# sndels/yuki

Measured on AMD Instinct MI355X. Metric: Mray/s (primary+secondary), Path integrator @1080p, higher is better.
Workload: dtype f32; 1 GPU; cfg3: city 40x20 displaced icospheres, 1,024,012 triangles, SAH BVH (max_shapes_in_node 1), Path 8 bounces, Stratified 8x8, 1920x1080; triangles=1024012, spp=64, max_depth=8, tiles=8160, partition=single GPU, frames_in_flight=2

## Files before the change

yuki_amd/csrc/yk_kernels.h:

```cpp
#pragma once
#include <hip/hip_runtime.h>

#include "yk_device.h"

namespace yk {

unsigned trace_block_size();
unsigned trace_spill_depth();
unsigned trace_top_nodes();
unsigned trace_top_nodes_any();
unsigned packet_blocks_per_cu();
void launch_trace_closest_packet(hipStream_t s, unsigned grid, const DevScene& sc, const float4* rayO, const float4* rayD, const unsigned* count_ptr,
                                 unsigned* head, int* hit_tri, unsigned long long* ray_counter, const float4* lean_origin = nullptr, CancelRef cancel = CancelRef{nullptr, nullptr});
void launch_trace_any_packet(hipStream_t s, unsigned grid, const DevScene& sc, const float4* shO, const float4* shD, const unsigned* slot_of,
                             const unsigned* count_ptr, unsigned* head, unsigned char* vis, unsigned long long* shadow_counter, CancelRef cancel = CancelRef{nullptr, nullptr});
unsigned trace_blocks_per_cu();

void launch_pixel_table(hipStream_t s, const yk_tile* tiles, const uint32_t* tile_offset, uint32_t n_tiles, uint32_t n_pixels, uint32_t* pixel_xy,
                        const uint16_t* tile_sample = nullptr, uint32_t* pixel_sample = nullptr);
void launch_pixel_table_one(hipStream_t s, const yk_tile& tile, uint32_t n_pixels, uint32_t* pixel_xy, uint32_t tile_sample, uint32_t* pixel_sample);
void launch_raygen(hipStream_t s, const DevCamera& cam, const RenderParams& prm, const uint32_t* pixel_xy, const uint32_t* pixel_sample, uint64_t work0,
                   uint32_t n, PathBuffers out, float4* sample_buf, unsigned* count, float4* lean_origin = nullptr, const uint4* pixel_aux = nullptr);
void launch_pixel_sampler(hipStream_t s, const SamplerCfg& cfg, const uint32_t* pixel_xy, uint32_t n_pixels, uint4* pixel_aux);
void launch_raygen_user(hipStream_t s, const RenderParams& prm, const float* o, const float* d, const uint16_t* pixel, const uint32_t* sample_index,
                        uint32_t dimension, uint32_t n, PathBuffers out, float4* sample_buf, uint32_t* pixel_xy, unsigned* ctrl);
void launch_trace_closest(hipStream_t s, unsigned grid, const DevScene& sc, const float4* rayO, const float4* rayD, const float* t_max_opt,
                          const unsigned* count_ptr, unsigned* head, int* hit_tri, float4* hit_out, uint4* stats_out, uint2* spill,
                          unsigned spill_stride, unsigned* ctrl, unsigned long long* ray_counter, const unsigned* cancel_host = nullptr);
void launch_whitted(hipStream_t s, unsigned grid, const DevScene& sc, const RenderParams& prm, const uint32_t* pixel_xy, const uint32_t* sample_index_tab,
                    PathBuffers cur, uint32_t n, float4* sample_buf, uint2* spill, unsigned spill_stride, unsigned* ctrl, unsigned long long* counters);
unsigned whitted_max_depth();
void launch_path_debug(hipStream_t s, unsigned grid, const DevScene& sc, const RenderParams& prm, const uint32_t* pixel_xy, const uint32_t* sample_index_tab,
                       PathBuffers cur, uint32_t n, float4* sample_buf, uint32_t* out_counts, float4* out_rays, unsigned ray_cap, uint32_t* out_n_rays,
                       float min_len, uint2* spill, unsigned spill_stride, unsigned* ctrl);
void launch_trace_any(hipStream_t s, unsigned grid, const DevScene& sc, const float4* shO, const float4* shD, const unsigned* slot_of,
                      const unsigned* count_ptr, unsigned* head, unsigned char* vis, uint2* spill, unsigned spill_stride, unsigned* ctrl,
                      unsigned long long* shadow_counter, const unsigned* cancel_host = nullptr);
void launch_shade(hipStream_t s, unsigned grid, const DevScene& sc, const RenderParams& prm, const uint32_t* pixel_xy, const uint32_t* sample_index_tab,
                  PathBuffers cur, PathBuffers nxt, const int* hit_tri, float4* pend, float4* shO, float4* shD, float4* shC, unsigned char* vis,
                  unsigned* shq, float4* shO2, float4* shD2, unsigned* shq2, unsigned* bc, unsigned split_delta, unsigned reorder, unsigned block_slots, unsigned sid_base, const float4* lean_origin);
void launch_accumulate(hipStream_t s, unsigned grid, const RenderParams& prm, PathBuffers cur, const float4* pend, const float4* shC,
                       const unsigned char* vis, unsigned nl, float4* sample_buf, const unsigned* bc, unsigned first, unsigned sid_base);
void launch_resolve(hipStream_t s, const float4* sample_buf, uint32_t n_pixels, uint32_t spp, float* out_rgb);
void launch_resolve_passes(hipStream_t s, const float4* sample_buf, uint32_t n_pixels, uint32_t n_passes, float* out_rgb, size_t pass_stride);
void launch_film_scatter(hipStream_t s, const uint32_t* pixel_xy, uint32_t n_pixels, const float* tile_rgb, uint32_t res_x, float* film_rgb, int accumulate,
                         uint32_t n_passes = 1, size_t pass_stride = 0);
void launch_debug_shade(hipStream_t s, const DevScene& sc, uint32_t integrator, PathBuffers cur, const int* hit_tri, const uint4* stats, uint32_t n,
                        float4* sample_buf);
void launch_device_math(hipStream_t s, int fn, size_t n, const float* a, const float* b, float* out);
void launch_sampler_sequence(hipStream_t s, const SamplerCfg& cfg, uint32_t px, uint32_t py, uint32_t sample_index, const uint8_t* dims, size_t n_draws,
                             float* out);
void launch_light_test(hipStream_t s, const DevLight& L, int index, size_t n, const float* p, const float* ng, const float* u, float* out);
void launch_bsdf_test(hipStream_t s, const Material& m, size_t n, const float* ng, const float* ns, const float* dpdu, const float* wo,
                      const float* wi_or_u, int sample, float* out);
void launch_pack_rays(hipStream_t s, size_t n, const float* o, const float* d, float4* rayO, float4* rayD);
void launch_pack_shadow_rays(hipStream_t s, size_t n, const float* o, const float* d, const float* t_max, const int* area_light, float4* shO,
                             float4* shD);
void launch_unpack_rays(hipStream_t s, size_t n, const float4* rayO, const float4* rayD, float* o, float* d);

}
```

yuki_amd/csrc/yk_kernels.hip:

```cpp
#include <hip/hip_runtime.h>

#include "yk_device.h"
#include "yk_geom.h"
#include "yk_kernels.h"
#include "yk_rng.h"
#include "yk_shade.h"
#include "yk_wave.h"

namespace yk {

__global__ void k_pixel_table(const yk_tile* tiles, const uint32_t* tile_offset, uint32_t n_tiles, uint32_t n_pixels,
                              uint32_t* pixel_xy, const uint16_t* tile_sample, uint32_t* pixel_sample) {
    uint32_t i = blockIdx.x * blockDim.x + threadIdx.x;
    if (i >= n_pixels) return;
    uint32_t lo = 0, hi = n_tiles;
    while (hi - lo > 1) {
        uint32_t mid = (lo + hi) >> 1;
        if (tile_offset[mid] <= i)
            lo = mid;
        else
            hi = mid;
    }
    yk_tile t = tiles[lo];
    uint32_t w = (uint32_t)t.x1 - t.x0;
    uint32_t r = i - tile_offset[lo];
    uint32_t x = t.x0 + r % w, y = t.y0 + r / w;
    pixel_xy[i] = x | (y << 16);
    if (tile_sample) pixel_sample[i] = tile_sample[lo];
}

__global__ void k_pixel_table_one(yk_tile t, uint32_t n_pixels, uint32_t* pixel_xy, uint32_t tile_sample, uint32_t* pixel_sample) {
    uint32_t i = blockIdx.x * blockDim.x + threadIdx.x;
    if (i >= n_pixels) return;
    uint32_t w = (uint32_t)t.x1 - t.x0;
    pixel_xy[i] = (t.x0 + i % w) | ((t.y0 + i / w) << 16);
    if (pixel_sample) pixel_sample[i] = tile_sample;
}

__global__ void k_pixel_sampler(SamplerCfg cfg, const uint32_t* pixel_xy, uint32_t n_pixels, uint4* pixel_aux) {
    uint32_t i = blockIdx.x * blockDim.x + threadIdx.x;
    if (i >= n_pixels) return;
    const uint32_t xy = pixel_xy[i];
    const PixelSampler ps = pixel_sampler(cfg, xy & 0xffffu, xy >> 16);
    pixel_aux[i] = make_uint4((unsigned)ps.stream, (unsigned)(ps.stream >> 32), ps.hash0, 0u);
}

__device__ __forceinline__ void camera_ray(const DevCamera& cam, float fx, float fy, V3& o, V3& d) {
    V3 p_camera = xf_point(cam.r2c, V3{fx, fy, 0.0f});
    V3 dir = normalize(p_camera);
    o = xf_point(cam.c2w, V3{0.0f, 0.0f, 0.0f});
    d = xf_vector(cam.c2w, dir);
}

__global__ void k_raygen(DevCamera cam, RenderParams prm, const uint32_t* pixel_xy, const uint32_t* pixel_sample, uint64_t work0, uint32_t n,
                         PathBuffers out, float4* sample_buf, unsigned* count, float4* lean_origin, const uint4* pixel_aux) {
    uint32_t i = blockIdx.x * blockDim.x + threadIdx.x;
    if (cancel_raised(prm.cancel)) return;
    if (i == 0) *count = n;
    if (i >= n) return;
    const uint32_t w = (uint32_t)(work0 + i);
    uint32_t pix, ks;
    split_sample_id(w, prm.spe, pix, ks);
    const uint32_t s = (pixel_sample ? pixel_sample[pix] : prm.sample_base) + ks;
    uint32_t xy = pixel_xy[pix];
    uint32_t px = xy & 0xffffu, py = xy >> 16;
    SamplerState st;
    float ux, uy;
    if (pixel_aux) {
        const uint4 a = pixel_aux[pix];
        PixelSampler ps;
        ps.stream = (u64)a.x | ((u64)a.y << 32);
        ps.hash0 = a.z;
        st = sampler_start_camera(prm.sampler, ps, px, py, s, ux, uy);
    } else {
        st = sampler_start(prm.sampler, px, py, s, 0);
        sampler_get_2d(prm.sampler, st, ux, uy);
    }
    V3 o, d;
    camera_ray(cam, (float)px + ux, (float)py + uy, o, d);
    if (lean_origin) {
        if (i == 0) *lean_origin = make_float4(o.x, o.y, o.z, __uint_as_float(0u));
    } else {
        out.rayO[i] = make_float4(o.x, o.y, o.z, __uint_as_float(0u));
        out.thru[i] = make_float4(1.0f, 1.0f, 1.0f, __uint_as_float(st.dimension));
    }
    out.rayD[i] = make_float4(d.x, d.y, d.z, __uint_as_float((uint32_t)w));
    out.rngs[i] = make_uint4((unsigned)st.rng.state, (unsigned)(st.rng.state >> 32), (unsigned)st.rng.inc, (unsigned)(st.rng.inc >> 32));
    if (prm.integrator != YK_INTEGRATOR_PATH || prm.max_depth == 0) sample_buf[w] = make_float4(0.0f, 0.0f, 0.0f, 0.0f);
}

__global__ void k_raygen_user(RenderParams prm, const float* ray_o, const float* ray_d, const uint16_t* pixel, const uint32_t* sample_index,
                              uint32_t dimension, uint32_t n, PathBuffers out, float4* sample_buf, uint32_t* pixel_xy, unsigned* count) {
    uint32_t i = blockIdx.x * blockDim.x + threadIdx.x;
    if (i == 0) *count = n;
    if (i >= n) return;
    uint32_t px = pixel[2 * i], py = pixel[2 * i + 1];
    pixel_xy[i] = px | (py << 16);
    SamplerState st = sampler_start(prm.sampler, px, py, sample_index[i], dimension);
    if (prm.sampler.kind == 1) st.dimension = dimension;
    out.rayO[i] = make_float4(ray_o[3 * i], ray_o[3 * i + 1], ray_o[3 * i + 2], __uint_as_float(0u));
    out.rayD[i] = make_float4(ray_d[3 * i], ray_d[3 * i + 1], ray_d[3 * i + 2], __uint_as_float(i));
    out.thru[i] = make_float4(1.0f, 1.0f, 1.0f, __uint_as_float(st.dimension));
    out.rngs[i] = make_uint4((unsigned)st.rng.state, (unsigned)(st.rng.state >> 32), (unsigned)st.rng.inc, (unsigned)(st.rng.inc >> 32));
    if (prm.integrator != YK_INTEGRATOR_PATH || prm.max_depth == 0) sample_buf[i] = make_float4(0.0f, 0.0f, 0.0f, 0.0f);
}

#ifndef SHADE_CAP
#define SHADE_CAP 335
#endif
#ifndef SHADE_CAPQ
#define SHADE_CAPQ 768
#endif
#ifndef SHADE_WIN
#define SHADE_WIN 8
#endif
#ifndef SHADE_MIN_WAVES
#define SHADE_MIN_WAVES 3
#endif
template <int CAP, int CAPQ> struct ShadeStaging {
    float4 pO[CAP], pD[CAP], pT[CAP];
    uint4 pR[CAP];
    float4 qO[CAPQ], qD[CAPQ];
    unsigned qS[CAPQ];
    unsigned fill_p, fill_q, gbase;
    unsigned q_delta;
    unsigned cancel;
    unsigned bucket[8];
    unsigned short order[SHADE_WIN * 256];
};

__device__ __forceinline__ unsigned block_append(bool want, unsigned* lds_fill) {
    unsigned long long mask = __ballot(want);
    unsigned total = (unsigned)__popcll(mask);
    unsigned prefix = (unsigned)__popcll(mask & ((1ull << lane_id()) - 1ull));
    unsigned base = 0;
    if (total && lane_id() == 0) base = atomicAdd(lds_fill, total);
    base = __shfl(base, 0);
    return base + prefix;
}

__device__ __forceinline__ unsigned valid_light_kind(const DevScene& sc, unsigned l) { return sc.lights[l].kind; }

#ifdef YK_SHADE_PROFILE
#include "../../tools/micro/shade_profile.h"
#else
#define YK_PROF_DECL
#define YK_PROF_STAMP(k)
#define YK_PROF_FLUSH
#endif

template <int BLOCK, int CAP, int CAPQ>
__global__ __launch_bounds__(BLOCK, SHADE_MIN_WAVES) void k_shade(DevScene sc, RenderParams prm, const uint32_t* pixel_xy, const uint32_t* sample_index_tab,
                                                 PathBuffers cur, PathBuffers nxt,
                                                 const int* hit_tri, float4* pend, float4* shO, float4* shD, float4* shC, unsigned char* vis,
                                                 unsigned* shq, float4* shO2, float4* shD2, unsigned* shq2, unsigned* bc, unsigned split_delta, unsigned reorder,
                                                 unsigned win_max, unsigned block_slots, unsigned sid_base, const float4* __restrict__ lean_origin) {
    const unsigned win_iters = min(win_max, max(1u, bc[0] / (BLOCK * block_slots)));
    static_assert(sizeof(ShadeStaging<CAP, CAPQ>) <= 53296, "k_shade: more LDS than the measured 53296 bytes per block (42 granules = 53760 cost the third block per CU)");
    __shared__ ShadeStaging<CAP, CAPQ> stg;
    const unsigned nl = sc.n_lights;
    unsigned* next_count = bc + YK_CTRL_STRIDE;
    unsigned* shq_count = bc + YK_CTRL_SHQ;
    if (threadIdx.x == 0) {
        stg.fill_p = 0;
        stg.fill_q = 0;
        stg.q_delta = 0;
        stg.cancel = cancel_raised(prm.cancel) ? 1u : 0u;
    }
    __syncthreads();
    const unsigned n = __builtin_amdgcn_readfirstlane((int)stg.cancel) ? 0u : bc[0];
    auto flush_q = [&](unsigned fill, unsigned delta) {
        if (threadIdx.x == 0) stg.gbase = atomicAdd(delta ? bc + YK_CTRL_SHQ2 : shq_count, fill);
        __syncthreads();
        const unsigned gb = stg.gbase;
        float4* dO = delta ? shO2 : shO;
        float4* dD = delta ? shD2 : shD;
        unsigned* dS = delta ? shq2 : shq;
        for (unsigned k = threadIdx.x; k < fill; k += BLOCK) {
            dO[gb + k] = stg.qO[k];
            dD[gb + k] = stg.qD[k];
            dS[gb + k] = stg.qS[k];
        }
        __syncthreads();
        if (threadIdx.x == 0) stg.fill_q = 0;
        __syncthreads();
    };
    auto flush_p = [&](unsigned fill) {
        if (threadIdx.x == 0) stg.gbase = atomicAdd(next_count, fill);
        __syncthreads();
        const unsigned gb = stg.gbase;
        for (unsigned k = threadIdx.x; k < fill; k += BLOCK) {
            nxt.rayO[gb + k] = stg.pO[k];
            nxt.rayD[gb + k] = stg.pD[k];
            nxt.thru[gb + k] = stg.pT[k];
            nxt.rngs[gb + k] = stg.pR[k];
        }
        __syncthreads();
        if (threadIdx.x == 0) stg.fill_p = 0;
        __syncthreads();
    };
    const bool per_iter = !split_delta && BLOCK * nl <= (unsigned)CAPQ;
    const unsigned WIN = win_iters * BLOCK;
    const unsigned n_win = (n + WIN - 1) / WIN;
    YK_PROF_DECL
    for (unsigned w = blockIdx.x; w < n_win; w += gridDim.x) {
      const unsigned wbase = w * WIN;
      unsigned n_sub = win_iters;
      YK_PROF_STAMP(0)
      if (reorder) {
        if (threadIdx.x < 8) stg.bucket[threadIdx.x] = 0;
        __syncthreads();
        unsigned key[SHADE_WIN], rank[SHADE_WIN];
#pragma unroll
        for (int k = 0; k < SHADE_WIN; ++k) {
            const unsigned i0 = wbase + k * BLOCK + threadIdx.x;
            const bool in = (unsigned)k < win_iters && i0 < n;
            const int t = in ? hit_tri[i0] : -1;
            key[k] = !in ? 7u : (t < 0 ? 6u : ((unsigned)t >> YK_HIT_KIND_SHIFT));
        }
#pragma unroll
        for (int k = 0; k < SHADE_WIN; ++k) {
            rank[k] = 0;
            if ((unsigned)k >= win_iters) continue;
            for (unsigned q = 0; q < 8; ++q) {
                const unsigned long long m = __ballot(key[k] == q);
                if (m == 0ull) continue;
                unsigned b0 = 0;
                if (lane_id() == 0) b0 = atomicAdd(&stg.bucket[q], (unsigned)__popcll(m));
                b0 = __shfl(b0, 0);
                if (key[k] == q) rank[k] = b0 + (unsigned)__popcll(m & ((1ull << lane_id()) - 1ull));
            }
        }
        __syncthreads();
        unsigned first[8];
        {
            unsigned acc = 0;
            for (unsigned q = 0; q < 8; ++q) {
                first[q] = acc;
                acc += stg.bucket[q];
            }
            n_sub = (acc - stg.bucket[7] + BLOCK - 1) / BLOCK;
        }
#pragma unroll
        for (int k = 0; k < SHADE_WIN; ++k)
            if ((unsigned)k < win_iters) stg.order[first[key[k]] + rank[k]] = (unsigned short)(k * BLOCK + threadIdx.x);
        __syncthreads();
      } else {
        const unsigned left = n - wbase;
        n_sub = left >= WIN ? win_iters : (left + BLOCK - 1) / BLOCK;
      }
      for (unsigned sub = 0; sub < n_sub; ++sub) {
        const unsigned i = wbase + (reorder ? (unsigned)stg.order[sub * BLOCK + threadIdx.x] : sub * BLOCK + threadIdx.x);
        const bool valid = i < n;
        bool alive = false;
        YK_PROF_STAMP(1)
        if (per_iter) {
            __syncthreads();
            const unsigned fq = stg.fill_q, fp = stg.fill_p, staged = stg.q_delta;
            __syncthreads();
            if (fq && fq + BLOCK * nl > CAPQ) flush_q(fq, staged);
            if (fp + BLOCK > CAP) flush_p(fp);
        }
        float4 nO = make_float4(0, 0, 0, 0), nD = nO, nT = nO;
        uint4 nR = make_uint4(0, 0, 0, 0);
        V3 o = V3{0, 0, 0}, d = V3{0, 0, 1};
        RGB beta = RGB{0, 0, 0};
        unsigned flags = 0, sid = 0, bounces = 0;
        bool specular_bounce = false, hit = false;
        SamplerState st;
        st.rng.state = 0;
        st.rng.inc = 1;
        st.px = st.py = st.sample_index = st.dimension = 0;
        PathVertex v;
        v.sf.p = v.sf.n = v.sf.ns = v.sf.dpdus = v.sf.wo = V3{0, 0, 1};
        v.sf.material = 0;
        v.sf.area_light = -1;
        v.sf.u = v.sf.v = 0.0f;
        v.mat.kind = MK_BLACK;
        v.fr.s = v.fr.t = v.fr.n = v.fr.ng = V3{0, 0, 1};
        v.wo = V3{0, 0, 1};
        if (valid) {
            float4 a, c;
            const float4 b = cur.rayD[i];
            if (lean_origin) {
                a = *lean_origin;
                c = make_float4(1.0f, 1.0f, 1.0f, __uint_as_float(2u));
            } else {
                a = cur.rayO[i];
                c = cur.thru[i];
            }
            uint4 r = cur.rngs[i];
            o = f4_xyz(a);
            d = f4_xyz(b);
            flags = __float_as_uint(a.w);
            sid = __float_as_uint(b.w);
            beta = RGB{c.x, c.y, c.z};
            bounces = flags & 0xffu;
            specular_bounce = (flags >> 8) & 1u;
            st = path_sampler(prm, pixel_xy, sample_index_tab, r, __float_as_uint(c.w), sid);
            int tri = hit_tri[i];
            hit = tri >= 0;
            if (hit) vertex_setup(sc, (uint32_t)tri & YK_HIT_PRIM_MASK, o, d, v);
        }
        YK_PROF_STAMP(2)
        const unsigned vs = YK_VIS_STRIDE(nl);
        unsigned vword = 0u;
        for (unsigned l = 0; l < nl; ++l) {
            const unsigned slot = i * nl + l, vslot = i * vs + l;
            NeeSample ne;
            ne.want = false;
            ne.contrib = RGB{0, 0, 0};
            ne.so = V3{0, 0, 0};
            ne.sd = V3{0, 0, 1};
            ne.al = -1;
            if (valid && hit) ne = vertex_light(sc, prm, st, l, v);
            const bool want = ne.want;
            if (vs == 4u)
                vword |= (want ? 1u : 0u) << (8u * l);
            else if (valid)
                vis[vslot] = want ? 1 : 0;
            if (!per_iter) {
                __syncthreads();
                const unsigned f = stg.fill_q, staged = stg.q_delta;
                const unsigned delta = (split_delta && valid_light_kind(sc, l) != YK_LIGHT_RECT) ? 1u : 0u;
                __syncthreads();
                if (f && (staged != delta || f + BLOCK > CAPQ)) flush_q(f, staged);
                if (threadIdx.x == 0) stg.q_delta = delta;
            }
            unsigned q = block_append(want, &stg.fill_q);
            if (want) {
                stg.qO[q] = make_float4(ne.so.x, ne.so.y, ne.so.z, 0.9999f);
                stg.qD[q] = make_float4(ne.sd.x, ne.sd.y, ne.sd.z, __uint_as_float((unsigned)ne.al));
                stg.qS[q] = vslot;
                shC[slot] = make_float4(ne.contrib.r, ne.contrib.g, ne.contrib.b, 0.0f);
            }
        }
        if (vs == 4u && valid) reinterpret_cast<unsigned*>(vis)[i] = vword;
        YK_PROF_STAMP(3)
        if (valid) {
            unsigned kind = 0;
            RGB term = RGB{0, 0, 0};
            if (!hit) {
                term = vertex_miss_term(sc, beta);
                kind = YK_PEND_MISS;
            } else {
                VertexEnd e = vertex_finish(sc, prm, st, v, beta, bounces, specular_bounce);
                term = e.term;
                kind = e.kind;
                alive = e.alive;
                if (e.sampled) {
                    nO = make_float4(e.no.x, e.no.y, e.no.z, __uint_as_float((bounces & 0xffu) | (specular_bounce ? 0x100u : 0u)));
                    nD = make_float4(e.wi.x, e.wi.y, e.wi.z, __uint_as_float(sid));
                    nT = make_float4(beta.r, beta.g, beta.b, __uint_as_float(st.dimension));
                    nR = make_uint4((unsigned)st.rng.state, (unsigned)(st.rng.state >> 32), (unsigned)st.rng.inc, (unsigned)(st.rng.inc >> 32));
                }
            }
            pend[i] = make_float4(term.r, term.g, term.b, __uint_as_float((kind << YK_PEND_KIND_SHIFT) | (sid - sid_base)));
        }
        YK_PROF_STAMP(4)
        if (!per_iter) {
            __syncthreads();
            const unsigned f = stg.fill_p;
            __syncthreads();
            if (f + BLOCK > CAP) flush_p(f);
        }
        unsigned j = block_append(alive, &stg.fill_p);
        if (alive) {
            stg.pO[j] = nO;
            stg.pD[j] = nD;
            stg.pT[j] = nT;
            stg.pR[j] = nR;
        }
        YK_PROF_STAMP(5)
      }
      if (reorder) __syncthreads();
    }
    YK_PROF_FLUSH
    __syncthreads();
    {
        const unsigned fq = stg.fill_q, fp = stg.fill_p;
        if (fq) flush_q(fq, stg.q_delta);
        if (fp) flush_p(fp);
    }
}

__global__ void k_accumulate(RenderParams prm, PathBuffers cur, const float4* pend, const float4* shC, const unsigned char* vis, unsigned nl,
                             float4* sample_buf, const unsigned* bc, unsigned first, unsigned sid_base) {
    const unsigned n = cancel_raised(prm.cancel) ? 0u : bc[0];
    for (unsigned i = blockIdx.x * blockDim.x + threadIdx.x; i < n; i += gridDim.x * blockDim.x) {
        float4 p = pend[i];
        const unsigned kind = __float_as_uint(p.w) >> YK_PEND_KIND_SHIFT;
        const unsigned sid = sid_base + (__float_as_uint(p.w) & YK_PEND_SID_MASK);
        RGB beta = RGB{1.0f, 1.0f, 1.0f};
        if (!first && !(kind & YK_PEND_MISS)) {
            const float4 c = cur.thru[i];
            beta = RGB{c.x, c.y, c.z};
        }
        RGB L = RGB{0.0f, 0.0f, 0.0f};
        if (!first) {
            const float4 acc = sample_buf[sid];
            L = RGB{acc.x, acc.y, acc.z};
        }
        RGB radiance = RGB{0.0f, 0.0f, 0.0f};
        if (!(kind & YK_PEND_MISS)) {
            const unsigned vs = YK_VIS_STRIDE(nl);
            const unsigned vword = vs == 4u ? reinterpret_cast<const unsigned*>(vis)[i] : 0u;
            for (unsigned l = 0; l < nl; ++l) {
                const unsigned slot = i * nl + l;
                const unsigned verdict = vs == 4u ? (vword >> (8u * l)) & 255u : (unsigned)vis[i * vs + l];
                if (verdict == 1u) {
                    float4 ct = shC[slot];
                    radiance = radiance + RGB{ct.x, ct.y, ct.z};
                }
            }
        }
        L = vertex_accumulate(prm, L, beta, radiance, RGB{p.x, p.y, p.z}, kind);
        sample_buf[sid] = make_float4(L.r, L.g, L.b, 0.0f);
    }
}

__global__ void k_resolve(const float4* sample_buf, uint32_t n_pixels, uint32_t spp, float* out_rgb) {
    uint32_t p = blockIdx.x * blockDim.x + threadIdx.x;
    if (p >= n_pixels) return;
    RGB color = RGB{0.0f, 0.0f, 0.0f};
    const float4* s = sample_buf + (size_t)p * spp;
    uint32_t k = 0;
    for (; k + 8 <= spp; k += 8) {
        float4 v[8];
#pragma unroll
        for (int j = 0; j < 8; ++j) v[j] = s[k + j];
#pragma unroll
        for (int j = 0; j < 8; ++j) color = color + RGB{v[j].x, v[j].y, v[j].z};
    }
    for (; k < spp; ++k) {
        float4 v = s[k];
        color = color + RGB{v.x, v.y, v.z};
    }
    color = color / (float)spp;
    out_rgb[3 * (size_t)p + 0] = color.r;
    out_rgb[3 * (size_t)p + 1] = color.g;
    out_rgb[3 * (size_t)p + 2] = color.b;
}

__global__ void k_resolve_passes(const float4* sample_buf, uint32_t n_pixels, uint32_t n_passes, float* out_rgb, size_t pass_stride) {
    const size_t i = (size_t)blockIdx.x * blockDim.x + threadIdx.x;
    if (i >= (size_t)n_pixels * n_passes) return;
    const uint32_t p = (uint32_t)(i / n_passes), k = (uint32_t)(i % n_passes);
    const float4 v = sample_buf[i];
    float* o = out_rgb + (size_t)k * pass_stride + 3 * (size_t)p;
    o[0] = v.x;
    o[1] = v.y;
    o[2] = v.z;
}

__global__ void k_film_scatter(const uint32_t* pixel_xy, uint32_t n_pixels, const float* tile_rgb, uint32_t res_x, float* film_rgb, int accumulate,
                               uint32_t n_passes, size_t pass_stride) {
    uint32_t p = blockIdx.x * blockDim.x + threadIdx.x;
    if (p >= n_pixels) return;
    uint32_t xy = pixel_xy[p];
    size_t dst = (size_t)(xy >> 16) * res_x + (xy & 0xffffu);
    if (accumulate) {
        float r = film_rgb[3 * dst + 0], g = film_rgb[3 * dst + 1], b = film_rgb[3 * dst + 2];
        for (uint32_t k = 0; k < n_passes; ++k) {
            const float* t = tile_rgb + (size_t)k * pass_stride + 3 * (size_t)p;
            r += t[0];
// ... 130 lines not shown
        out[8 * i + 4] = s.f.g;
        out[8 * i + 5] = s.f.b;
        out[8 * i + 6] = s.pdf;
        out[8 * i + 7] = (float)s.type;
    }
}

__global__ void k_light_test(DevLight L, int index, size_t n, const float* p, const float* ng, const float* u, float* out) {
    size_t i = blockIdx.x * (size_t)blockDim.x + threadIdx.x;
    if (i >= n) return;
    const V3 sp = ld3(p, (uint32_t)i), nn = ld3(ng, (uint32_t)i);
    LightSample ls = sample_light(L, index, sp, u[2 * i], u[2 * i + 1]);
    V3 offset = nn * 0.001f;
    V3 so = dot(ls.p1 - sp, nn) > 0.0f ? sp + offset : sp - offset;
    V3 sd = ls.p1 - so;
    float* o = out + 18 * i;
    o[0] = ls.l.x; o[1] = ls.l.y; o[2] = ls.l.z;
    o[3] = ls.li.r; o[4] = ls.li.g; o[5] = ls.li.b;
    o[6] = ls.pdf;
    o[7] = ls.has_vis ? 1.0f : 0.0f;
    o[8] = (float)ls.area_light;
    o[9] = ls.p1.x; o[10] = ls.p1.y; o[11] = ls.p1.z;
    o[12] = so.x; o[13] = so.y; o[14] = so.z;
    o[15] = sd.x; o[16] = sd.y; o[17] = sd.z;
}

__global__ void k_pack_rays(size_t n, const float* o, const float* d, float4* rayO, float4* rayD) {
    size_t i = blockIdx.x * (size_t)blockDim.x + threadIdx.x;
    if (i >= n) return;
    rayO[i] = make_float4(o[3 * i], o[3 * i + 1], o[3 * i + 2], 0.0f);
    rayD[i] = make_float4(d[3 * i], d[3 * i + 1], d[3 * i + 2], 0.0f);
}
__global__ void k_pack_shadow_rays(size_t n, const float* o, const float* d, const float* t_max, const int* area_light, float4* shO, float4* shD) {
    size_t i = blockIdx.x * (size_t)blockDim.x + threadIdx.x;
    if (i >= n) return;
    shO[i] = make_float4(o[3 * i], o[3 * i + 1], o[3 * i + 2], t_max[i]);
    shD[i] = make_float4(d[3 * i], d[3 * i + 1], d[3 * i + 2], __uint_as_float((unsigned)(area_light ? area_light[i] : -1)));
}
__global__ void k_unpack_rays(size_t n, const float4* rayO, const float4* rayD, float* o, float* d) {
    size_t i = blockIdx.x * (size_t)blockDim.x + threadIdx.x;
    if (i >= n) return;
    float4 a = rayO[i], b = rayD[i];
    o[3 * i] = a.x; o[3 * i + 1] = a.y; o[3 * i + 2] = a.z;
    d[3 * i] = b.x; d[3 * i + 1] = b.y; d[3 * i + 2] = b.z;
}

#ifdef YK_SHADE_PROFILE
}
extern "C" int yk_debug_shade_profile(unsigned long long* out8, int reset) {
    unsigned long long zero[8] = {0, 0, 0, 0, 0, 0, 0, 0};
    (void)hipDeviceSynchronize();
    int rc = (int)hipMemcpyFromSymbol(out8, HIP_SYMBOL(yk::yk_shade_prof), sizeof(zero));
    if (reset) rc |= (int)hipMemcpyToSymbol(HIP_SYMBOL(yk::yk_shade_prof), zero, sizeof(zero));
    return rc;
}
namespace yk {
#endif

static inline unsigned blocks_for(size_t n, unsigned bs) { return (unsigned)((n + bs - 1) / bs); }

void launch_pixel_table(hipStream_t s, const yk_tile* tiles, const uint32_t* tile_offset, uint32_t n_tiles, uint32_t n_pixels, uint32_t* pixel_xy,
                        const uint16_t* tile_sample, uint32_t* pixel_sample) {
    if (!n_pixels) return;
    hipLaunchKernelGGL(k_pixel_table, dim3(blocks_for(n_pixels, 256)), dim3(256), 0, s, tiles, tile_offset, n_tiles, n_pixels, pixel_xy, tile_sample,
                       pixel_sample);
}
void launch_pixel_table_one(hipStream_t s, const yk_tile& tile, uint32_t n_pixels, uint32_t* pixel_xy, uint32_t tile_sample, uint32_t* pixel_sample) {
    if (!n_pixels) return;
    hipLaunchKernelGGL(k_pixel_table_one, dim3(blocks_for(n_pixels, 256)), dim3(256), 0, s, tile, n_pixels, pixel_xy, tile_sample, pixel_sample);
}
void launch_pixel_sampler(hipStream_t s, const SamplerCfg& cfg, const uint32_t* pixel_xy, uint32_t n_pixels, uint4* pixel_aux) {
    if (!n_pixels) return;
    hipLaunchKernelGGL(k_pixel_sampler, dim3(blocks_for(n_pixels, 256)), dim3(256), 0, s, cfg, pixel_xy, n_pixels, pixel_aux);
}
void launch_raygen(hipStream_t s, const DevCamera& cam, const RenderParams& prm, const uint32_t* pixel_xy, const uint32_t* pixel_sample, uint64_t work0,
                   uint32_t n, PathBuffers out, float4* sample_buf, unsigned* count, float4* lean_origin, const uint4* pixel_aux) {
    hipLaunchKernelGGL(k_raygen, dim3(blocks_for(n, 256)), dim3(256), 0, s, cam, prm, pixel_xy, pixel_sample, work0, n, out, sample_buf, count, lean_origin, pixel_aux);
}
void launch_raygen_user(hipStream_t s, const RenderParams& prm, const float* o, const float* d, const uint16_t* pixel, const uint32_t* sample_index,
                        uint32_t dimension, uint32_t n, PathBuffers out, float4* sample_buf, uint32_t* pixel_xy, unsigned* ctrl) {
    hipLaunchKernelGGL(k_raygen_user, dim3(blocks_for(n, 256)), dim3(256), 0, s, prm, o, d, pixel, sample_index, dimension, n, out, sample_buf,
                       pixel_xy, ctrl);
}
void launch_shade(hipStream_t s, unsigned grid, const DevScene& sc, const RenderParams& prm, const uint32_t* pixel_xy, const uint32_t* sample_index_tab,
                  PathBuffers cur, PathBuffers nxt,
                  const int* hit_tri, float4* pend, float4* shO, float4* shD, float4* shC, unsigned char* vis, unsigned* shq, float4* shO2,
                  float4* shD2, unsigned* shq2, unsigned* bc, unsigned split_delta, unsigned reorder, unsigned block_slots, unsigned sid_base, const float4* lean_origin) {
    hipLaunchKernelGGL((k_shade<256, SHADE_CAP, SHADE_CAPQ>), dim3(grid), dim3(256), 0, s, sc, prm, pixel_xy, sample_index_tab, cur, nxt, hit_tri, pend, shO, shD, shC, vis, shq,
                       shO2, shD2, shq2, bc, split_delta, reorder, (unsigned)SHADE_WIN, block_slots, sid_base, lean_origin);
}
void launch_accumulate(hipStream_t s, unsigned grid, const RenderParams& prm, PathBuffers cur, const float4* pend, const float4* shC,
                       const unsigned char* vis, unsigned nl, float4* sample_buf, const unsigned* bc, unsigned first, unsigned sid_base) {
    hipLaunchKernelGGL(k_accumulate, dim3(grid), dim3(256), 0, s, prm, cur, pend, shC, vis, nl, sample_buf, bc, first, sid_base);
}
void launch_resolve(hipStream_t s, const float4* sample_buf, uint32_t n_pixels, uint32_t spp, float* out_rgb) {
    if (!n_pixels) return;
    hipLaunchKernelGGL(k_resolve, dim3(blocks_for(n_pixels, 256)), dim3(256), 0, s, sample_buf, n_pixels, spp, out_rgb);
}
void launch_resolve_passes(hipStream_t s, const float4* sample_buf, uint32_t n_pixels, uint32_t n_passes, float* out_rgb, size_t pass_stride) {
    if (!n_pixels) return;
    hipLaunchKernelGGL(k_resolve_passes, dim3(blocks_for((size_t)n_pixels * n_passes, 256)), dim3(256), 0, s, sample_buf, n_pixels, n_passes, out_rgb, pass_stride);
}
void launch_film_scatter(hipStream_t s, const uint32_t* pixel_xy, uint32_t n_pixels, const float* tile_rgb, uint32_t res_x, float* film_rgb, int accumulate,
                         uint32_t n_passes, size_t pass_stride) {
    if (!n_pixels) return;
    hipLaunchKernelGGL(k_film_scatter, dim3(blocks_for(n_pixels, 256)), dim3(256), 0, s, pixel_xy, n_pixels, tile_rgb, res_x, film_rgb, accumulate, n_passes, pass_stride);
}
void launch_debug_shade(hipStream_t s, const DevScene& sc, uint32_t integrator, PathBuffers cur, const int* hit_tri, const uint4* stats, uint32_t n,
                        float4* sample_buf) {
    hipLaunchKernelGGL(k_debug_shade, dim3(blocks_for(n, 256)), dim3(256), 0, s, sc, integrator, cur, hit_tri, stats, n, sample_buf);
}
void launch_device_math(hipStream_t s, int fn, size_t n, const float* a, const float* b, float* out) {
    hipLaunchKernelGGL(k_device_math, dim3(blocks_for(n, 256)), dim3(256), 0, s, fn, n, a, b, out);
}
void launch_sampler_sequence(hipStream_t s, const SamplerCfg& cfg, uint32_t px, uint32_t py, uint32_t sample_index, const uint8_t* dims, size_t n_draws,
                             float* out) {
    hipLaunchKernelGGL(k_sampler_sequence, dim3(1), dim3(64), 0, s, cfg, px, py, sample_index, dims, n_draws, out);
}
void launch_light_test(hipStream_t s, const DevLight& L, int index, size_t n, const float* p, const float* ng, const float* u, float* out) {
    hipLaunchKernelGGL(k_light_test, dim3(blocks_for(n, 256)), dim3(256), 0, s, L, index, n, p, ng, u, out);
}
void launch_bsdf_test(hipStream_t s, const Material& m, size_t n, const float* ng, const float* ns, const float* dpdu, const float* wo,
                      const float* wi_or_u, int sample, float* out) {
    hipLaunchKernelGGL(k_bsdf_test, dim3(blocks_for(n, 256)), dim3(256), 0, s, m, n, ng, ns, dpdu, wo, wi_or_u, sample, out);
}
void launch_pack_rays(hipStream_t s, size_t n, const float* o, const float* d, float4* rayO, float4* rayD) {
    hipLaunchKernelGGL(k_pack_rays, dim3(blocks_for(n, 256)), dim3(256), 0, s, n, o, d, rayO, rayD);
}
void launch_pack_shadow_rays(hipStream_t s, size_t n, const float* o, const float* d, const float* t_max, const int* area_light, float4* shO,
                             float4* shD) {
    hipLaunchKernelGGL(k_pack_shadow_rays, dim3(blocks_for(n, 256)), dim3(256), 0, s, n, o, d, t_max, area_light, shO, shD);
}
void launch_unpack_rays(hipStream_t s, size_t n, const float4* rayO, const float4* rayD, float* o, float* d) {
    hipLaunchKernelGGL(k_unpack_rays, dim3(blocks_for(n, 256)), dim3(256), 0, s, n, rayO, rayD, o, d);
}

}
```

yuki_amd/csrc/yk_render.cpp:

```cpp
#include <hip/hip_runtime.h>

#include <algorithm>
#include <chrono>
#include <cstdio>
#include <cstdlib>
#include <cstring>
#include <mutex>
#include <string>
#include <thread>
#include <vector>

#include "yk_internal.h"
#ifdef YK_EXPERIMENT_SORT
#include "../../tools/micro/ray_sort_experiment.h"
#endif
#ifdef YK_EXPERIMENT_GRAPH
#include "../../tools/micro/graph_replay_experiment.h"
#endif

unsigned* error_block(yk_context* ctx) { return reinterpret_cast<unsigned*>(ctx->counters.as<unsigned long long>() + 16); }
CancelRef cancel_ref(yk_context* ctx) { return CancelRef{ctx->cancel_host_dev, ctx->cancel_host_dev ? error_block(ctx) + YK_CTRL_CANCELLED : nullptr}; }

yk_status ensure_work_buffers(yk_context* ctx, WorkSet& ws, size_t paths, unsigned n_lights, unsigned n_delta_lights) {
    HIP_TRY(ctx, ctx->counters.ensure(YK_COUNTER_BYTES));
// ... 27 lines not shown
unsigned trace_grid(const yk_context* ctx) { return (unsigned)ctx->n_cu * trace_blocks_per_cu(); }

yk_status ensure_spill(yk_context* ctx, WorkSet& ws) {
    size_t threads = (size_t)trace_grid(ctx) * trace_block_size();
    HIP_TRY(ctx, ws.spill.ensure(threads * trace_spill_depth() * 8));
    HIP_TRY(ctx, ws.spill_side.ensure(threads * trace_spill_depth() * 8));
    return YK_OK;
}

PathBuffers path_buffers(WorkSet& ws, int which) {
    PathBuffers p;
    p.rayO = ws.path[which][0].as<float4>();
    p.rayD = ws.path[which][1].as<float4>();
    p.thru = ws.path[which][2].as<float4>();
    p.rngs = ws.path[which][3].as<uint4>();
    return p;
}

yk_status make_params(yk_context* ctx, const yk_sampler_desc* smp, const yk_integrator_desc* integ, RenderParams& prm) {
    if (!smp || !integ) return fail(ctx, YK_ERR_INVALID_ARGUMENT, "null sampler/integrator");
    std::memset(&prm, 0, sizeof(prm));
    prm.sampler.kind = smp->kind;
    prm.sampler.nx = smp->nx;
    prm.sampler.ny = smp->kind == YK_SAMPLER_UNIFORM ? 1 : smp->ny;
    prm.sampler.jitter = smp->jitter;
    prm.sampler.seed = smp->seed;
    if (smp->kind > 1 || prm.sampler.nx == 0 || prm.sampler.ny == 0) return fail(ctx, YK_ERR_INVALID_ARGUMENT, "bad sampler");
    uint64_t spp = (uint64_t)prm.sampler.nx * prm.sampler.ny;
    if (spp > 0xFFFFu) return fail(ctx, YK_ERR_INVALID_ARGUMENT, "samples per pixel exceed u16 (integrators/mod.rs:139)");
    prm.sampler.spp = (unsigned)spp;
    prm.spe = (unsigned)spp;
    prm.max_depth = integ->max_depth;
    prm.has_clamp = integ->has_clamp;
    prm.clamp = integ->indirect_clamp;
    prm.integrator = integ->kind;
    if (integ->kind == YK_INTEGRATOR_WHITTED && integ->max_depth > whitted_max_depth())
        return fail(ctx, YK_ERR_UNSUPPORTED, "Whitted: max_depth above 16 is not supported on the device");
    if (integ->kind > YK_INTEGRATOR_SHADING_UVS) return fail(ctx, YK_ERR_INVALID_ARGUMENT, "bad integrator kind");
    return YK_OK;
}


bool packet_kernel_traces_bounce(const yk_context* ctx, const yk_scene* scene, unsigned b) {
    return b < (unsigned)ctx->packet_bounces && scene->bvh->depth <= 64;
}

void run_bounces(yk_context* ctx, WorkSet& ws, hipStream_t st, const yk_scene* scene, const RenderParams& prm, const uint32_t* pixel_xy,
                        const uint32_t* sample_index_tab, float4* sample_buf, KernelTimer& kt, unsigned long long* counters, bool coherent,
                        uint32_t n_paths, uint32_t sid_base, bool lean_camera_bounce, uint32_t* n_shadow_launches) {
    unsigned* ctrl = ws.ctrl.as<unsigned>();
    unsigned* errblk = error_block(ctx);
    const DevScene ds = dev_scene_for(scene, n_paths);
    auto fit = [](unsigned full, uint64_t items) { return (unsigned)std::min<uint64_t>(full, std::max<uint64_t>(1, (items + 255) / 256)); };
    const uint64_t n_shadow_max = (uint64_t)n_paths * std::max(1u, scene->n_lights);
    const unsigned tg = fit(trace_grid(ctx), n_paths), tg_any = fit(trace_grid(ctx), n_shadow_max);
    const unsigned pg_full = (unsigned)ctx->n_cu * packet_blocks_per_cu();
    const unsigned pg = fit(pg_full, n_paths), pg_any = fit(pg_full, n_shadow_max);
    static const unsigned shade_bpc = std::getenv("YK_SHADE_BPC") ? (unsigned)std::atoi(std::getenv("YK_SHADE_BPC")) : 256u;
    const unsigned sg = fit((unsigned)ctx->n_cu * shade_bpc, n_paths);
    const unsigned spill_stride = trace_grid(ctx) * trace_block_size();
    unsigned cur = 0;
    const bool overlap = ctx->overlap_shadow != 0 && ws.side != nullptr;
    hipStream_t sb = overlap ? ws.side : st;
    for (unsigned b = 0; b < prm.max_depth; ++b) {
        PathBuffers pc = path_buffers(ws, (int)cur), pn = path_buffers(ws, (int)(cur ^ 1u));
        const bool packet = coherent && packet_kernel_traces_bounce(ctx, scene, b);
        const float4* lean_origin = (b == 0 && lean_camera_bounce) ? reinterpret_cast<const float4*>(ctrl + YK_CTRL_CAM_O) : nullptr;
        const bool packet_shadow = coherent && b < (unsigned)ctx->packet_shadow_bounces && scene->bvh->depth <= 64 && scene->n_delta_lights > 0;
        const bool split = packet_shadow && scene->n_lights > scene->n_delta_lights;
        const bool all_delta = packet_shadow && !split;
        unsigned* bc = ctrl + YK_CTRL_BOUNCE(b);
        int e = kt.begin(st);
        if (packet)
            launch_trace_closest_packet(st, pg, ds, lean_origin ? nullptr : pc.rayO, pc.rayD, bc, bc + YK_CTRL_HEAD, ws.hit.as<int>(), counters, lean_origin, prm.cancel);
        else {
            launch_trace_closest(st, tg, ds, pc.rayO, pc.rayD, nullptr, bc, bc + YK_CTRL_HEAD, ws.hit.as<int>(), nullptr, nullptr,
                                 ws.spill.as<uint2>(), spill_stride, errblk, counters, prm.cancel.host);
        }
        kt.end(e, 0, st);
        if (overlap && b > 0) (void)hipStreamWaitEvent(st, ws.ev_acc, 0);
        e = kt.begin(st);
        launch_shade(st, sg, ds, prm, pixel_xy, sample_index_tab, pc, pn, ws.hit.as<int>(), ws.pend.as<float4>(), ws.shO.as<float4>(),
                     ws.shD.as<float4>(), ws.shC.as<float4>(), ws.vis.as<unsigned char>(), ws.shq.as<unsigned>(), ws.shO2.as<float4>(),
                     ws.shD2.as<float4>(), ws.shq2.as<unsigned>(), bc, split ? 1u : 0u, (b > 0 && ctx->shade_reorder) ? 1u : 0u, 3u * (unsigned)ctx->n_cu, sid_base, lean_origin);
        kt.end(e, 2, st);
#ifdef YK_EXPERIMENT_SORT
        YK_SORT_AFTER_SHADE
#endif
        if (overlap) {
            (void)hipEventRecord(ws.ev_shade, st);
            (void)hipStreamWaitEvent(sb, ws.ev_shade, 0);
        }
        e = kt.begin(sb);
        uint2* any_spill = (overlap ? ws.spill_side : ws.spill).as<uint2>();
        if (all_delta) {
            launch_trace_any_packet(sb, pg_any, ds, ws.shO.as<float4>(), ws.shD.as<float4>(), ws.shq.as<unsigned>(), bc + YK_CTRL_SHQ,
                                    bc + YK_CTRL_HEAD + 1, ws.vis.as<unsigned char>(), counters + 1, prm.cancel);
        } else {
            launch_trace_any(sb, tg_any, ds, ws.shO.as<float4>(), ws.shD.as<float4>(), ws.shq.as<unsigned>(), bc + YK_CTRL_SHQ,
                             bc + YK_CTRL_HEAD + 1, ws.vis.as<unsigned char>(), any_spill, spill_stride, errblk, counters + 1, prm.cancel.host);
            if (split && n_shadow_launches) ++*n_shadow_launches;
            if (split)
                launch_trace_any_packet(sb, pg_any, ds, ws.shO2.as<float4>(), ws.shD2.as<float4>(), ws.shq2.as<unsigned>(), bc + YK_CTRL_SHQ2,
                                        bc + YK_CTRL_HEAD + 2, ws.vis.as<unsigned char>(), counters + 1, prm.cancel);
        }
        kt.end(e, 1, sb);
        if (n_shadow_launches) ++*n_shadow_launches;
        launch_accumulate(sb, sg, prm, pc, ws.pend.as<float4>(), ws.shC.as<float4>(), ws.vis.as<unsigned char>(), ds.n_lights, sample_buf, bc, b == 0 ? 1u : 0u, sid_base);
        if (overlap) (void)hipEventRecord(ws.ev_acc, sb);
        if (kt.on && std::getenv("YK_DEBUG_BOUNCES")) {
            unsigned h[YK_CTRL_STRIDE + 1];
            (void)hipStreamSynchronize(st);
            (void)hipStreamSynchronize(sb);
            (void)hipMemcpy(h, bc, sizeof(h), hipMemcpyDeviceToHost);
            float tt = 0, ts = 0, th = 0;
            (void)hipEventElapsedTime(&tt, ctx->ev_pool[kt.spans[0].back().first], ctx->ev_pool[kt.spans[0].back().second]);
            (void)hipEventElapsedTime(&ts, ctx->ev_pool[kt.spans[1].back().first], ctx->ev_pool[kt.spans[1].back().second]);
            (void)hipEventElapsedTime(&th, ctx->ev_pool[kt.spans[2].back().first], ctx->ev_pool[kt.spans[2].back().second]);
            std::fprintf(stderr, "bounce %u: rays %u trace %.3f ms (%.0f Mray/s) | shadow rays %u %.3f ms (%.0f Mray/s) | shade %.3f ms | survivors %u\n", b, h[0],
                         tt, h[0] / (tt * 1e3), h[YK_CTRL_SHQ] + h[YK_CTRL_SHQ2], ts, (h[YK_CTRL_SHQ] + h[YK_CTRL_SHQ2]) / (ts * 1e3), th, h[YK_CTRL_STRIDE]);
        }
        cur ^= 1u;
    }
    if (overlap) (void)hipStreamWaitEvent(st, ws.ev_acc, 0);
}

static double now_ms() { return std::chrono::duration<double, std::milli>(std::chrono::steady_clock::now().time_since_epoch()).count(); }
static const bool g_debug_cancel = std::getenv("YK_DEBUG_CANCEL") != nullptr;

static void raise_cancel(yk_context* ctx, bool from_render_thread = true) {
    if (!ctx->cancel_host) return;
    const double t0 = g_debug_cancel ? now_ms() : 0.0;
    ctx->cancel_raised.store(true, std::memory_order_release);
    __atomic_store_n(ctx->cancel_host, 1u, __ATOMIC_RELEASE);
    if (from_render_thread && !ctx->cancel_stream) ctx->want_cancel_stream = true;
    if (from_render_thread && ctx->cancel_stream && ctx->counters.p)
        (void)hipMemcpyAsync(error_block(ctx) + YK_CTRL_CANCELLED, ctx->cancel_host + 16, 4, hipMemcpyHostToDevice, ctx->cancel_stream);
    if (g_debug_cancel) std::fprintf(stderr, "[yk cancel] raise: %s, %.3f ms\n", ctx->cancel_stream ? "host word + device word" : "host word only (first interruption)", now_ms() - t0);
}

static yk_status clear_cancel(yk_context* ctx) {
    if (!ctx->cancel_host || !ctx->cancel_raised.load(std::memory_order_acquire)) return YK_OK;
    HIP_TRY(ctx, hipStreamSynchronize(ctx->stream));
    if (ctx->cancel_stream) HIP_TRY(ctx, hipStreamSynchronize(ctx->cancel_stream));
    for (WorkSet& w : ctx->ws) {
        if (w.stream && w.stream != ctx->stream) HIP_TRY(ctx, hipStreamSynchronize(w.stream));
        if (w.side) HIP_TRY(ctx, hipStreamSynchronize(w.side));
    }
    __atomic_store_n(ctx->cancel_host, 0u, __ATOMIC_RELEASE);
    ctx->cancel_raised.store(false, std::memory_order_release);
    if (ctx->want_cancel_stream && !ctx->cancel_stream) {
        if (hipStreamCreateWithFlags(&ctx->cancel_stream, hipStreamNonBlocking) != hipSuccess) ctx->cancel_stream = nullptr;
        ctx->want_cancel_stream = false;
    }
    return YK_OK;
}

static bool poll_until(yk_context* ctx, hipEvent_t done, yk_cancel_fn cancel, void* user) {
    while (hipEventQuery(done) == hipErrorNotReady) {
        if (cancel(user)) {
            raise_cancel(ctx);
            return true;
        }
        std::this_thread::sleep_for(std::chrono::microseconds(100));
    }
    return false;
}
// ... 675 lines not shown
```

Baseline: 2295 Mray/s.

## Write continuation rays directly to global via per-iteration block reservation, freeing LDS

The shade kernel stops staging surviving continuation rays in shared memory and flushing them in batches. Each iteration now reserves slots with a block-wide ballot and one atomic, then every thread writes its ray straight to the next-bounce buffers. This frees roughly 21 KB of LDS per block, so the launch bound rises to four waves and the grid sizing uses a computed blocks-per-CU. In exchange there is one global atomic and extra barriers per iteration, and the global writes are smaller and less coalesced than the old batched flush.

```diff
diff --git a/yuki_amd/csrc/yk_kernels.h b/yuki_amd/csrc/yk_kernels.h
--- a/yuki_amd/csrc/yk_kernels.h
+++ b/yuki_amd/csrc/yk_kernels.h
@@ -15,6 +15,7 @@
 void launch_trace_any_packet(hipStream_t s, unsigned grid, const DevScene& sc, const float4* shO, const float4* shD, const unsigned* slot_of,
                              const unsigned* count_ptr, unsigned* head, unsigned char* vis, unsigned long long* shadow_counter, CancelRef cancel = CancelRef{nullptr, nullptr});
 unsigned trace_blocks_per_cu();
+unsigned shade_blocks_per_cu();
 
 void launch_pixel_table(hipStream_t s, const yk_tile* tiles, const uint32_t* tile_offset, uint32_t n_tiles, uint32_t n_pixels, uint32_t* pixel_xy,
                         const uint16_t* tile_sample = nullptr, uint32_t* pixel_sample = nullptr);
diff --git a/yuki_amd/csrc/yk_kernels.hip b/yuki_amd/csrc/yk_kernels.hip
--- a/yuki_amd/csrc/yk_kernels.hip
+++ b/yuki_amd/csrc/yk_kernels.hip
@@ -105,9 +105,6 @@
     if (prm.integrator != YK_INTEGRATOR_PATH || prm.max_depth == 0) sample_buf[i] = make_float4(0.0f, 0.0f, 0.0f, 0.0f);
 }
 
-#ifndef SHADE_CAP
-#define SHADE_CAP 335
-#endif
 #ifndef SHADE_CAPQ
 #define SHADE_CAPQ 768
 #endif
@@ -115,14 +112,14 @@
 #define SHADE_WIN 8
 #endif
 #ifndef SHADE_MIN_WAVES
-#define SHADE_MIN_WAVES 3
+#define SHADE_MIN_WAVES 4
 #endif
-template <int CAP, int CAPQ> struct ShadeStaging {
-    float4 pO[CAP], pD[CAP], pT[CAP];
-    uint4 pR[CAP];
+template <int CAPQ> struct ShadeStaging {
     float4 qO[CAPQ], qD[CAPQ];
     unsigned qS[CAPQ];
-    unsigned fill_p, fill_q, gbase;
+    unsigned fill_q, gbase;
+    unsigned wave_alive[2][4];
+    unsigned pbase;
     unsigned q_delta;
     unsigned cancel;
     unsigned bucket[8];
@@ -149,20 +146,20 @@
 #define YK_PROF_FLUSH
 #endif
 
-template <int BLOCK, int CAP, int CAPQ>
+template <int BLOCK, int CAPQ>
 __global__ __launch_bounds__(BLOCK, SHADE_MIN_WAVES) void k_shade(DevScene sc, RenderParams prm, const uint32_t* pixel_xy, const uint32_t* sample_index_tab,
                                                  PathBuffers cur, PathBuffers nxt,
                                                  const int* hit_tri, float4* pend, float4* shO, float4* shD, float4* shC, unsigned char* vis,
                                                  unsigned* shq, float4* shO2, float4* shD2, unsigned* shq2, unsigned* bc, unsigned split_delta, unsigned reorder,
                                                  unsigned win_max, unsigned block_slots, unsigned sid_base, const float4* __restrict__ lean_origin) {
     const unsigned win_iters = min(win_max, max(1u, bc[0] / (BLOCK * block_slots)));
-    static_assert(sizeof(ShadeStaging<CAP, CAPQ>) <= 53296, "k_shade: more LDS than the measured 53296 bytes per block (42 granules = 53760 cost the third block per CU)");
-    __shared__ ShadeStaging<CAP, CAPQ> stg;
+    static_assert(BLOCK == 256, "k_shade: four waves per block (ShadeStaging::wave_alive, shade_blocks_per_cu)");
+    static_assert(sizeof(ShadeStaging<CAPQ>) <= 40960, "k_shade: more LDS than 32 granules of 1280 bytes per block: the fourth block no longer fits a CU's 160 KB");
+    __shared__ ShadeStaging<CAPQ> stg;
     const unsigned nl = sc.n_lights;
     unsigned* next_count = bc + YK_CTRL_STRIDE;
     unsigned* shq_count = bc + YK_CTRL_SHQ;
     if (threadIdx.x == 0) {
-        stg.fill_p = 0;
         stg.fill_q = 0;
         stg.q_delta = 0;
         stg.cancel = cancel_raised(prm.cancel) ? 1u : 0u;
@@ -185,23 +182,25 @@
         if (threadIdx.x == 0) stg.fill_q = 0;
         __syncthreads();
     };
-    auto flush_p = [&](unsigned fill) {
-        if (threadIdx.x == 0) stg.gbase = atomicAdd(next_count, fill);
+    auto reserve_p = [&](bool alive, unsigned parity) -> unsigned {
+        const unsigned long long mask = __ballot(alive);
+        const unsigned wave = threadIdx.x >> 6;
+        if (lane_id() == 0) stg.wave_alive[parity][wave] = (unsigned)__popcll(mask);
         __syncthreads();
-        const unsigned gb = stg.gbase;
-        for (unsigned k = threadIdx.x; k < fill; k += BLOCK) {
-            nxt.rayO[gb + k] = stg.pO[k];
-            nxt.rayD[gb + k] = stg.pD[k];
-            nxt.thru[gb + k] = stg.pT[k];
-            nxt.rngs[gb + k] = stg.pR[k];
+        if (threadIdx.x == 0) {
+            const unsigned total = stg.wave_alive[parity][0] + stg.wave_alive[parity][1] + stg.wave_alive[parity][2] + stg.wave_alive[parity][3];
+            if (total) stg.pbase = atomicAdd(next_count, total);
         }
         __syncthreads();
-        if (threadIdx.x == 0) stg.fill_p = 0;
-        __syncthreads();
+        unsigned slot = stg.pbase + (unsigned)__popcll(mask & ((1ull << lane_id()) - 1ull));
+        for (unsigned k = 0; k < 3; ++k)
+            if (k < wave) slot += stg.wave_alive[parity][k];
+        return slot;
     };
     const bool per_iter = !split_delta && BLOCK * nl <= (unsigned)CAPQ;
     const unsigned WIN = win_iters * BLOCK;
     const unsigned n_win = (n + WIN - 1) / WIN;
+    unsigned parity = 0;
     YK_PROF_DECL
     for (unsigned w = blockIdx.x; w < n_win; w += gridDim.x) {
       const unsigned wbase = w * WIN;
@@ -256,10 +255,9 @@
         YK_PROF_STAMP(1)
         if (per_iter) {
             __syncthreads();
-            const unsigned fq = stg.fill_q, fp = stg.fill_p, staged = stg.q_delta;
+            const unsigned fq = stg.fill_q, staged = stg.q_delta;
             __syncthreads();
             if (fq && fq + BLOCK * nl > CAPQ) flush_q(fq, staged);
-            if (fp + BLOCK > CAP) flush_p(fp);
         }
         float4 nO = make_float4(0, 0, 0, 0), nD = nO, nT = nO;
         uint4 nR = make_uint4(0, 0, 0, 0);
@@ -358,18 +356,13 @@
             pend[i] = make_float4(term.r, term.g, term.b, __uint_as_float((kind << YK_PEND_KIND_SHIFT) | (sid - sid_base)));
         }
         YK_PROF_STAMP(4)
-        if (!per_iter) {
-            __syncthreads();
-            const unsigned f = stg.fill_p;
-            __syncthreads();
-            if (f + BLOCK > CAP) flush_p(f);
-        }
-        unsigned j = block_append(alive, &stg.fill_p);
+        const unsigned j = reserve_p(alive, parity);
+        parity ^= 1u;
         if (alive) {
-            stg.pO[j] = nO;
-            stg.pD[j] = nD;
-            stg.pT[j] = nT;
-            stg.pR[j] = nR;
+            nxt.rayO[j] = nO;
+            nxt.rayD[j] = nD;
+            nxt.thru[j] = nT;
+            nxt.rngs[j] = nR;
         }
         YK_PROF_STAMP(5)
       }
@@ -378,9 +371,8 @@
     YK_PROF_FLUSH
     __syncthreads();
     {
-        const unsigned fq = stg.fill_q, fp = stg.fill_p;
+        const unsigned fq = stg.fill_q;
         if (fq) flush_q(fq, stg.q_delta);
-        if (fp) flush_p(fp);
     }
 }
 
@@ -677,11 +669,18 @@
     hipLaunchKernelGGL(k_raygen_user, dim3(blocks_for(n, 256)), dim3(256), 0, s, prm, o, d, pixel, sample_index, dimension, n, out, sample_buf,
                        pixel_xy, ctrl);
 }
+unsigned shade_blocks_per_cu() {
+    const unsigned granules = ((unsigned)sizeof(ShadeStaging<SHADE_CAPQ>) + 1279u) / 1280u;
+    const unsigned by_lds = 128u / granules;
+    const unsigned by_waves = (unsigned)SHADE_MIN_WAVES;
+    return by_lds < by_waves ? by_lds : by_waves;
+}
+
 void launch_shade(hipStream_t s, unsigned grid, const DevScene& sc, const RenderParams& prm, const uint32_t* pixel_xy, const uint32_t* sample_index_tab,
                   PathBuffers cur, PathBuffers nxt,
                   const int* hit_tri, float4* pend, float4* shO, float4* shD, float4* shC, unsigned char* vis, unsigned* shq, float4* shO2,
                   float4* shD2, unsigned* shq2, unsigned* bc, unsigned split_delta, unsigned reorder, unsigned block_slots, unsigned sid_base, const float4* lean_origin) {
-    hipLaunchKernelGGL((k_shade<256, SHADE_CAP, SHADE_CAPQ>), dim3(grid), dim3(256), 0, s, sc, prm, pixel_xy, sample_index_tab, cur, nxt, hit_tri, pend, shO, shD, shC, vis, shq,
+    hipLaunchKernelGGL((k_shade<256, SHADE_CAPQ>), dim3(grid), dim3(256), 0, s, sc, prm, pixel_xy, sample_index_tab, cur, nxt, hit_tri, pend, shO, shD, shC, vis, shq,
                        shO2, shD2, shq2, bc, split_delta, reorder, (unsigned)SHADE_WIN, block_slots, sid_base, lean_origin);
 }
 void launch_accumulate(hipStream_t s, unsigned grid, const RenderParams& prm, PathBuffers cur, const float4* pend, const float4* shC,
diff --git a/yuki_amd/csrc/yk_render.cpp b/yuki_amd/csrc/yk_render.cpp
--- a/yuki_amd/csrc/yk_render.cpp
+++ b/yuki_amd/csrc/yk_render.cpp
@@ -133,7 +133,7 @@
         e = kt.begin(st);
         launch_shade(st, sg, ds, prm, pixel_xy, sample_index_tab, pc, pn, ws.hit.as<int>(), ws.pend.as<float4>(), ws.shO.as<float4>(),
                      ws.shD.as<float4>(), ws.shC.as<float4>(), ws.vis.as<unsigned char>(), ws.shq.as<unsigned>(), ws.shO2.as<float4>(),
-                     ws.shD2.as<float4>(), ws.shq2.as<unsigned>(), bc, split ? 1u : 0u, (b > 0 && ctx->shade_reorder) ? 1u : 0u, 3u * (unsigned)ctx->n_cu, sid_base, lean_origin);
+                     ws.shD2.as<float4>(), ws.shq2.as<unsigned>(), bc, split ? 1u : 0u, (b > 0 && ctx->shade_reorder) ? 1u : 0u, shade_blocks_per_cu() * (unsigned)ctx->n_cu, sid_base, lean_origin);
         kt.end(e, 2, st);
 #ifdef YK_EXPERIMENT_SORT
         YK_SORT_AFTER_SHADE
```

Measured after the change: 2215 Mray/s. 3.5% lower.
